# fenghansen/YOND_public

Hardware: AMD Instinct MI355X
Metric: Bayer megapixels/sec end-to-end (NLE+VST+denoise+iVST) (higher is better)
Workload: dtype f32 (3x3 convolutions: f32 operands as two f16 halves -- 22-23 significant bits -- on the f16 MFMA, 3 products per f32 product, f32 accumulate; per-layer error vs float64 asserted <= 2x the f32 direct kernel's and <= 2e-5 of max|ref| (tests/test_hip_conv.py; measured 1.3e-6 vs 1.5e-6), whole frame v

## Files before the change

yond_public_amd/csrc/common.h:

```cpp
#pragma once
#include <hip/hip_runtime.h>
#include <stdint.h>
#include "../../include/yond_hip.h"

#ifdef YOND_EXPERIMENTS
#include <stdlib.h>
static inline long yond_exp_long(const char* name, long dflt) {
    const char* e = getenv(name);
    return e ? atol(e) : dflt;
}
#else
#define yond_exp_long(name, dflt) (dflt)
#endif

typedef float f32x16 __attribute__((ext_vector_type(16)));
typedef float f32x4 __attribute__((ext_vector_type(4)));
typedef float f32x2 __attribute__((ext_vector_type(2)));

#define YOND_LAUNCH_CHECK()                          \
    do {                                             \
        hipError_t e__ = hipGetLastError();          \
        if (e__ != hipSuccess) return (int)e__;      \
    } while (0)

struct YondRange {
    int pos = 0;
    unsigned neg = 0;
    __device__ __forceinline__ void add(const f32x4& v) {
        const int b0 = __float_as_int(v[0]), b1 = __float_as_int(v[1]), b2 = __float_as_int(v[2]), b3 = __float_as_int(v[3]);
        pos = max(max(max(pos, b0), b1), max(b2, b3));
        neg = max(max(max(neg, (unsigned)b0), (unsigned)b1), max((unsigned)b2, (unsigned)b3));
    }
    __device__ __forceinline__ bool at_most(float limit) const {
        return pos <= __float_as_int(limit) && neg <= (0x80000000u | (unsigned)__float_as_int(limit));
    }
    __device__ __forceinline__ bool below(float limit) const {
        return pos < __float_as_int(limit) && neg < (0x80000000u | (unsigned)__float_as_int(limit));
    }
};

__device__ __forceinline__ float silu_f(float x) { return x / (1.0f + expf(-x)); }

__device__ __forceinline__ int reflect101(int i, int n) {
    if (n == 1) return 0;
    const int period = 2 * (n - 1);
    i %= period;
    if (i < 0) i += period;
    return i >= n ? period - i : i;
}

__device__ __forceinline__ float wave_max(float v) {
#pragma unroll
    for (int o = 32; o > 0; o >>= 1) v = fmaxf(v, __shfl_xor(v, o));
    return v;
}

__device__ __forceinline__ double wave_sum(double v) {
#pragma unroll
    for (int o = 32; o > 0; o >>= 1) v += __shfl_xor(v, o);
    return v;
}

template <int I>
struct IntC {
// ... 10 lines not shown
```

yond_public_amd/csrc/conv_split.hip:

```cpp
#include "conv_split_kernel.h"

SPLIT_GROUP_K1S2(SPLIT_EXTERN)
SPLIT_GROUP_S1_64(SPLIT_EXTERN)
SPLIT_GROUP_S1_32(SPLIT_EXTERN)
SPLIT_GROUP_HALF(SPLIT_EXTERN)
SPLIT_GROUP_HALF128(SPLIT_EXTERN)
SPLIT_GROUP_HALF_TALL(SPLIT_EXTERN)
SPLIT_GROUP_FOLD(SPLIT_EXTERN)
SPLIT_GROUP_FOLD_S2(SPLIT_EXTERN)
SPLIT_GROUP_FOLD_K1(SPLIT_EXTERN)
SPLIT_GROUP_FOLD_NHWC(SPLIT_EXTERN)
SPLIT_GROUP_K1_D2(SPLIT_EXTERN)
SPLIT_GROUP_OSP(SPLIT_EXTERN)
SPLIT_GROUP_ISP(SPLIT_EXTERN)
SPLIT_GROUP_ISP_OSP(SPLIT_EXTERN)
SPLIT_GROUP_ISP_K1S2(SPLIT_EXTERN)
SPLIT_GROUP_K1_SUB2(SPLIT_EXTERN)
SPLIT_GROUP_WRES(SPLIT_EXTERN)
SPLIT_GROUP_D2(SPLIT_EXTERN)
SPLIT_GROUP_H_OSP(SPLIT_EXTERN)
SPLIT_GROUP_H_ISP_OSP(SPLIT_EXTERN)
SPLIT_GROUP_H_ISP_O4(SPLIT_EXTERN)
SPLIT_GROUP_H_K1S2(SPLIT_EXTERN)
SPLIT_GROUP_H_D2(SPLIT_EXTERN)
// ... 220 lines not shown
            if (half128s2) {
                if (!tall) return YOND_EUNSUPPORTED;
                return d.dst2 ? YOND_EUNSUPPORTED : launch_split<2, 8, 128, 2, 1, 2, false, false, false, 2>(d, st);
            }
            if (tall) return d.dst2 ? launch_split<2, 8, 64, 2, 1, 2, false, false, false, 2, false, false, true>(d, st) : launch_split<2, 8, 64, 2, 1, 2, false, false, false, 2>(d, st);
            return d.dst2 ? launch_split<2, 4, 64, 1, 1, 2, false, false, false, 2, false, false, true>(d, st) : launch_split<2, 4, 64, 1, 1, 2, false, false, false, 2>(d, st);
        }
#ifdef YOND_EXPERIMENTS
        if (isp && parts == 2 && yond_exp_long("YOND_SPLIT_S2_ROLES", 0) != 0)
            return d.dst2 ? launch_split<2, 4, 64, 2, 2, 2, false, false, false, 2, false, false, true, 0, 8, 1>(d, st) : launch_split<2, 4, 64, 2, 2, 2, false, false, false, 2, false, false, false, 0, 8, 1>(d, st);
        if (isp && parts == 2 && yond_exp_long("YOND_SPLIT_S2_W4", 0) != 0)
            return d.dst2 ? launch_split<2, 4, 64, 2, 2, 2, false, false, false, 2, false, false, true, 0, 4>(d, st) : launch_split<2, 4, 64, 2, 2, 2, false, false, false, 2, false, false, false, 0, 4>(d, st);
#endif
        if (isp && d.dst2) return launch_split<2, 4, 64, 1, 2, 2, false, false, false, 2, false, false, true>(d, st);
        if (isp) return launch_split<2, 4, 64, 1, 2, 2, false, false, false, 2>(d, st);
        if (!isp && parts == 2 && d.Wo <= 16 && !d.src1 && !d.res && !d.in_fmt && !d.out_fmt && yond_exp_long("YOND_SPLIT_FOLD", 1) != 0) {
            const int f = d.Wo <= 8 ? 4 : 2;
            const long long subs = (long long)d.N * ((d.Ho + 3) / 4) * ((d.Wo + 32 / f - 1) / (32 / f));
            const long long tiles_f = (long long)(d.Cout / 64) * ((subs + f - 1) / f), tiles = (long long)(d.Cout / 64) * ((d.Ho + 3) / 4) * d.N;
            if ((tiles_f + 255) / 256 < (tiles + 255) / 256)
                return f == 2 ? launch_split<2, 4, 64, 1, 2, 2, false, false, false, 0, false, false, false, 2>(d, st) : launch_split<2, 4, 64, 1, 2, 2, false, false, false, 0, false, false, false, 4>(d, st);
        }
        return parts == 2 ? launch_split<2, 4, 64, 1, 2, 2, false>(d, st) : launch_split<2, 4, 64, 1, 1, 2, false>(d, st);
    }
    if (d.Ho != d.H || d.Wo != d.W) return YOND_EINVAL;
    if (d.out4_dst && (tn != 32 || (parts != 2 && !isp))) return YOND_EUNSUPPORTED;
    if (op4) return YOND_EUNSUPPORTED;
    long long tiles12 = (long long)(d.Cout / 64) * ((d.Wo + 31) / 32) * ((d.Ho + 11) / 12) * d.N;
    {
        const long long tiles8 = (long long)(d.Cout / 64) * ((d.Wo + 31) / 32) * ((d.Ho + 7) / 8) * d.N;
        const long long r12 = (tiles12 + 255) / 256, r8 = (tiles8 + 255) / 256;
        if (8000 * r8 < 10044 * r12) tiles12 = 0;
    }
    const bool wres = parts == 2 && tn == 32 && d.Cout == 32 && d.C0 + d.C1 == 32 && yond_exp_long("YOND_SPLIT_WRES", 1) != 0;
#ifdef YOND_EXPERIMENTS
    const bool w4 = wres && (long long)((d.Wo + 31) / 32) * ((d.Ho + 7) / 8) * d.N >= 2048 && yond_exp_long("YOND_SPLIT_L0_W4", 0) != 0;
    if (w4 && isp && osp && !d.out4_dst) return launch_split<1, 8, 32, 2, 2, 2, false, false, false, true, true, false, false, 0, 4>(d, st);
    if (w4 && isp && !osp && d.out4_dst) return launch_split<1, 8, 32, 2, 2, 2, false, true, false, true, false, false, false, 0, 4>(d, st);
    if (w4 && !isp && osp && d.pre_act && !d.out4_dst) return launch_split<1, 8, 32, 2, 2, 2, true, false, false, false, true, false, false, 0, 4>(d, st);
#endif
    if (wres && isp && osp && !d.out4_dst) return launch_split<1, 16, 32, 2, 2, 2, false, false, false, true, true>(d, st);
    if (wres && isp && !osp && d.out4_dst) return launch_split<1, 16, 32, 2, 2, 2, false, true, false, true, false>(d, st);
    if (wres && !isp && osp && d.pre_act && !d.out4_dst) return launch_split<1, 16, 32, 2, 2, 2, true, false, false, false, true>(d, st);
    if ((isp || osp) && parts == 1) {
        if (osp && d.out4_dst) return YOND_EUNSUPPORTED;
        if (!isp && !(osp && d.pre_act)) return YOND_EUNSUPPORTED;
        if (isp && !osp) return (d.out4_dst && tn == 32) ? launch_split<1, 16, 32, 2, 1, 3, false, true, false, true>(d, st) : YOND_EUNSUPPORTED;
        if (half128) return isp ? launch_split<1, 8, 128, 2, 1, 3, false, false, false, true, true>(d, st) : launch_split<1, 8, 128, 2, 1, 3, true, false, false, false, true>(d, st);
        const bool t4_64 = tn == 64 && (long long)(d.Cout / 64) * ((d.Wo + 31) / 32) * ((d.Ho + 15) / 16) * d.N >= 256;
        const bool t4_32 = tn == 32 && (long long)((d.Wo + 31) / 32) * ((d.Ho + 31) / 32) * d.N >= 256;
        if (isp) {
            if (t4_64) return launch_split<1, 16, 64, 4, 1, 2, false, false, false, true, true>(d, st);
            if (t4_32) return launch_split<1, 32, 32, 4, 1, 2, false, false, false, true, true>(d, st);
            if (tn == 64 && tiles12 >= 256) return launch_split<1, 12, 64, 3, 1, 2, false, false, false, true, true>(d, st);
            if (tn == 64) return launch_split<1, 8, 64, 2, 1, 3, false, false, false, true, true>(d, st);
            return launch_split<1, 16, 32, 2, 1, 3, false, false, false, true, true>(d, st);
        }
        if (t4_64) return launch_split<1, 16, 64, 4, 1, 2, true, false, false, false, true>(d, st);
        if (tn == 64 && tiles12 >= 256) return launch_split<1, 12, 64, 3, 1, 2, true, false, false, false, true>(d, st);
        if (tn == 64) return launch_split<1, 8, 64, 2, 1, 3, true, false, false, false, true>(d, st);
        return launch_split<1, 16, 32, 2, 1, 3, true, false, false, false, true>(d, st);
    }
    if (isp || osp) {
        if (osp && d.out4_dst) return YOND_EUNSUPPORTED;
        int fold = 0;
        if (osp && (isp || d.pre_act) && tn == 64 && parts == 2 && d.Wo <= 16 && d.Wo == d.W && d.Ho == d.H && !d.src1 && yond_exp_long("YOND_SPLIT_FOLD", 1) != 0) {
            const int f = d.Wo <= 8 ? 4 : 2;
            const long long subs = (long long)d.N * ((d.Ho + 3) / 4) * ((d.Wo + 32 / f - 1) / (32 / f));
            const long long tiles_f = (long long)(d.Cout / 64) * ((subs + f - 1) / f), tiles8 = (long long)(d.Cout / 64) * ((d.Ho + 7) / 8) * d.N;
            const bool fits = (long long)d.H * d.W * (d.C0 > d.Cout ? d.C0 : d.Cout) * 4 * f < (1LL << 31);
            if (fits && 2 * ((tiles_f + 255) / 256) < 3 * ((tiles8 + 255) / 256)) fold = f;
        }
        if (isp && osp) {
            if (fold == 2) return launch_split<1, 4, 64, 1, 2, 3, false, false, false, true, true, false, false, 2>(d, st);
            if (fold == 4) return launch_split<1, 4, 64, 1, 2, 3, false, false, false, true, true, false, false, 4>(d, st);
            if (tn == 64 && tiles12 >= 256) return launch_split<1, 12, 64, 3, 2, 2, false, false, false, true, true>(d, st);
            if (tn == 64) return launch_split<1, 8, 64, 2, 2, 3, false, false, false, true, true>(d, st);
            return launch_split<1, 16, 32, 2, 2, 3, false, false, false, true, true>(d, st);
        }
        if (osp) {
            if (fold == 2) return launch_split<1, 4, 64, 1, 2, 3, true, false, false, false, true, false, false, 2>(d, st);
            if (fold == 4) return launch_split<1, 4, 64, 1, 2, 3, true, false, false, false, true, false, false, 4>(d, st);
            if (tn == 64 && tiles12 >= 256) return d.pre_act ? launch_split<1, 12, 64, 3, 2, 2, true, false, false, false, true>(d, st) : launch_split<1, 12, 64, 3, 2, 2, false, false, false, false, true>(d, st);
            if (tn == 64) return d.pre_act ? launch_split<1, 8, 64, 2, 2, 3, true, false, false, false, true>(d, st) : launch_split<1, 8, 64, 2, 2, 3, false, false, false, false, true>(d, st);
            return d.pre_act ? launch_split<1, 16, 32, 2, 2, 3, true, false, false, false, true>(d, st) : launch_split<1, 16, 32, 2, 2, 3, false, false, false, false, true>(d, st);
        }
        if (tn == 64 && tiles12 >= 256) return launch_split<1, 12, 64, 3, 2, 2, false, false, false, true>(d, st);
        if (tn == 64) return launch_split<1, 8, 64, 2, 2, 3, false, false, false, true>(d, st);
        if (d.out4_dst) return launch_split<1, 16, 32, 2, 2, 3, false, true, false, true>(d, st);
        return launch_split<1, 16, 32, 2, 2, 3, false, false, false, true>(d, st);
    }
    if (half128) {
        if (d.Ho != d.H || d.Wo != d.W) return YOND_EINVAL;
        long long t12 = (long long)(d.Cout / 128) * ((d.Wo + 31) / 32) * ((d.Ho + 11) / 12) * d.N;
        const long long t8 = (long long)(d.Cout / 128) * ((d.Wo + 31) / 32) * ((d.Ho + 7) / 8) * d.N;
        if (8000 * ((t8 + 255) / 256) < 10044 * ((t12 + 255) / 256)) t12 = 0;
        if (t12 >= 256) return d.pre_act ? launch_split<1, 12, 128, 3, 1, 2, true>(d, st) : launch_split<1, 12, 128, 3, 1, 2, false>(d, st);
        return d.pre_act ? launch_split<1, 8, 128, 2, 1, 3, true>(d, st) : launch_split<1, 8, 128, 2, 1, 3, false>(d, st);
    }
    if (tn == 64) {
        const bool th12 = tiles12 >= 256;
        if (parts == 2 && !d.pre_act && !d.src1 && !d.in_fmt && !d.out_fmt && !d.res_fmt && !d.out4_dst && !(d.ebatch && (d.escale || d.eshift)) && d.Wo <= 16 &&
            yond_exp_long("YOND_SPLIT_FOLD", 1) != 0) {
            const int f = d.Wo <= 8 ? 4 : 2;
// ... 20 lines not shown
```

yond_public_amd/csrc/conv_split_kernel.h:

```cpp
#pragma once
#include "common.h"
#include <cstdlib>

typedef _Float16 f16x8 __attribute__((ext_vector_type(8)));
typedef _Float16 f16x4 __attribute__((ext_vector_type(4)));

#ifndef SPLIT_DBG
#define SPLIT_DBG 0
#endif
#if SPLIT_DBG
static __device__ unsigned long long g_split_dbg[2][64][12];
#ifdef SPLIT_DBG_READER
extern "C" int SPLIT_DBG_READER(unsigned long long* host) {
    return (int)hipMemcpyFromSymbol(host, HIP_SYMBOL(g_split_dbg), sizeof(g_split_dbg));
}
#endif
#define SDBG(slot)                                                                                  \
    do {                                                                                            \
        if (blockIdx.x == 0 && (wave == 0 || wave == 4) && lane == 0 && dbg_step < 64)              \
            g_split_dbg[wave >> 2][dbg_step][slot] = __builtin_readcyclecounter();                  \
    } while (0)
#else
#define SDBG(slot) do {} while (0)
#endif
// ... 45 lines not shown
    static constexpr int NDI = (NDS + NWAVE - 1) / NWAVE;
    static_assert(NWB == 2 || NWB == 3, "two or three weight buffers");
    static_assert(!K1 || (STRIDE == 1 && PIX_ITEMS % NT == 0), "1x1 mode: whole chunks per pass of the staging threads");
    static_assert((NWAVE == 8 || NWAVE == 4) && RG * NCW == NWC && NW >= 1 && NW * NCW * 32 == TN, "wave grid does not cover the tile");
    static_assert(!ROLES || (NWAVE == 8 && !K1 && FOLD == 0), "role split: eight waves, the 3x3 forms");
    static_assert(FOLD == 0 || FOLD == 2 || FOLD == 4, "folded tiles: two or four sub-tiles");
};

constexpr int split_gcd(int a, int b) { return b == 0 ? a : split_gcd(b, a % b); }
constexpr int split_pairs(int mw, int stride, int r) {
    int n = 0;
    for (int m = 0; m < mw; ++m) n += (r - m * stride >= 0 && r - m * stride <= 2) ? 1 : 0;
    return n;
}
__device__ __forceinline__ float split_silu(float x) {
    return x * __builtin_amdgcn_rcpf(1.0f + __builtin_amdgcn_exp2f(x * -1.44269504088896341f));
}
template <int N>
__device__ __forceinline__ void split_barrier_keep_loads() { asm volatile("s_waitcnt vmcnt(%0) lgkmcnt(0)\n\ts_barrier" ::"n"(N) : "memory"); }

template <int STRIDE, int TH, int TN, int MW, int PARTS, int NWB, bool PRE, bool O4 = false, bool K1 = false, int ISPM = 0, bool OSP = false, bool S2 = false, bool D2 = false, int FOLD = 0, int NWAVE = 8, int ROLES = 0>
__global__ __launch_bounds__(64 * NWAVE, (NWAVE == 4 && STRIDE == 1) ? 2 : 1) void conv_split_kernel(const YondConvDesc d) {
    using C = SplitCfg<STRIDE, TH, TN, MW, PARTS, NWB, K1, FOLD, NWAVE, ROLES>;
    static_assert(!ROLES || (ISPM == 2 && !OSP && !O4 && !PRE), "role split: the register-staged split-plane input (stride 2)");
    static_assert(!FOLD || (!O4 && !S2 && ((!K1 && STRIDE == 1 && ISPM != 2 && OSP) || (STRIDE == 2 && (ISPM == 2 || (ISPM == 0 && !PRE && !D2))) || (K1 && ISPM == 2) || (!K1 && STRIDE == 1 && ISPM == 0 && !OSP && !PRE))),
                  "folded tiles: the split-plane data flow's kernels (3x3 stride 1: LDS-DMA or register-staged input, split-plane store; stride 2 and the decoder GEMM: register-staged split planes) "
                  "and the plain [N][H][W][C] 3x3 layer (training, UNetSeeInDark)");
    constexpr bool ISP = ISPM == 1, ISR = ISPM == 2;
    static_assert(ISPM == 0 || !PRE, "split-plane input: the producer applied the activation");
    static_assert(!OSP || (!O4 && !K1 && STRIDE == 1), "split-plane output: 3x3 stride-1 layers");
    static_assert(!S2 || (K1 && ISPM == 2 && TN == 64), "two sub-positions per tile: the decoder GEMM with register-staged split planes");
    static_assert(!D2 || (!OSP && !O4 && ((!K1 && STRIDE == 2) || (K1 && ISPM == 2 && !S2 && TN == 64))), "second output: the stride-2 layers and the decoder GEMM at split precision");
    constexpr int NACC = PARTS;
    constexpr int IPP = ISR ? 2 * PARTS : 4;
    constexpr int PIX_ITEMS = C::IH * C::IW * IPP;
    constexpr int NITEM = C::NPT * PIX_ITEMS;
    static_assert(!K1 || PIX_ITEMS % C::NTS == 0, "1x1 mode: whole chunks per pass of the staging threads");
    constexpr int NIN = ISP ? 0 : (NITEM + C::NTS - 1) / C::NTS;
    constexpr int NINA = NIN > 0 ? NIN : 1;
    constexpr int NDI = ISP ? C::NDI : 0;
    constexpr int KD = K1 ? PIX_ITEMS / C::NTS : NIN;
    constexpr int DPER = C::WPP / split_gcd(C::WPP, NWAVE);
    constexpr int NG = ISP ? (NDI < DPER ? NDI : DPER) : KD;
    constexpr int NOPS = C::NWT + NIN + NDI;
    constexpr int KEEP = (ISP || ROLES) ? (C::WAHEAD == 2 ? C::NWT_MIN : 0) : (C::WAHEAD == 2 ? NIN + C::NWT_MIN : NIN);
    extern __shared__ __attribute__((aligned(16))) float smem[];

    const int tid = threadIdx.x, lane = tid & 63, wave = tid >> 6;
    const int stid = ROLES ? tid - C::NTS : tid;
    const bool consumer = !ROLES || __builtin_amdgcn_readfirstlane(wave) < C::NWC;
    const int li = lane & 31, lh = lane >> 5;
    constexpr int FSW = FOLD ? 32 / FOLD : 32;
    const int fsub = FOLD ? li / FSW : 0, fcol = FOLD ? li % FSW : li, flds = (FOLD && !K1) ? li + (STRIDE == 2 ? 1 : 2) * fsub : li;
    const int rg = wave % C::RG, cg = wave / C::RG;

    const int nct = d.Cout / TN;
    const bool computes = d.Cout > 0;
    const int fnsx = (d.Wo + FSW - 1) / FSW, fnsy = (d.Ho + TH - 1) / TH;
    const int fper = fnsy * fnsx, fsubs = d.N * fper;
    struct FGeo { int n, oy0, ox0; };
    auto fold_geo = [&](int u) {
        FGeo g;
        const bool ok = u < fsubs;
        const int uu = ok ? u : fsubs - 1;
        g.n = uu / fper;
        const int r = uu - g.n * fper, ry = r / fnsx;
// ... 4 lines not shown
    const int ntx = FOLD ? (fsubs + FOLD - 1) / FOLD : (d.Wo + 31) / 32, nty = FOLD ? 1 : (d.Ho + TH - 1) / TH;
    const int Neff = FOLD ? 1 : d.N;
    const int tiles_per_img = nct * ntx * nty;
    const int total = tiles_per_img * Neff;
    const int G = gridDim.x;
    const int lslot = (G % 8 == 0) ? (blockIdx.x % 8) * (G / 8) + blockIdx.x / 8 : blockIdx.x;
    const int Cin = d.C0 + d.C1;
    const int nchunk = Cin / C::KSTEP;
    const int Cr = K1 ? d.Cout / 4 : d.Cout;
    const int cpb = S2 ? Cr / 32 : 1;
    auto k1_sp = [&](int ct, int cu) -> int {
        if constexpr (S2) return 2 * (ct / cpb) + ((cu >> 5) & 1);
        return cu / Cr;
    };
    auto k1_cb = [&](int ct, int cu) -> int {
        if constexpr (S2) return (ct % cpb) * 32 + (cu & 31);
        return cu % Cr;
    };
    const int my_sl = stid & (IPP - 1);
    const int my_plane = (my_sl >> 1) * PARTS * C::PLANE + (my_sl & 1) * 2;

    int in_lds[NINA];
#pragma unroll
    for (int k = 0; k < NIN; ++k) {
        const int it = stid + k * C::NTS;
        const int pt = it / PIX_ITEMS;
        const int pix = (it % PIX_ITEMS) / IPP;
        const int py = pix / C::IW, px = pix % C::IW;
        const int lp = (STRIDE == 2) ? py * C::TWP + (px & 1) * C::HALF + (px >> 1) : py * C::TWP + px;
        in_lds[k] = my_plane + (it < NITEM ? pt * 2 * PARTS * C::PLANE + lp * 4 : C::IH * C::TWP * 4);
        if constexpr (ISR) in_lds[k] = my_sl * C::PLANE + (it < NITEM ? pt * 2 * PARTS * C::PLANE + lp * 4 : C::IH * C::TWP * 4);
    }

    struct Tile {
        int ct, n, ox0, oy0;
        int fu0;
        int goff[NG];
        int goff1[K1 ? NG : 1];
    };
    const int wave_s = __builtin_amdgcn_readfirstlane(wave);
    const int PS0 = yond_sp_plane_units(d.H, d.W);
    const int PS1 = K1 ? yond_sp_plane_units(2 * d.H, 2 * d.W) : PS0;
    struct Cur { int tile, ch, ct, tx, ty, n; };
    int g_ct, g_tx, g_ty, g_n;
    {
        int b = G;
        g_ct = b % nct; b /= nct;
        g_tx = b % ntx; b /= ntx;
        g_ty = b % nty; g_n = b / nty;
    }
    auto cursor_at = [&](int t) {
        Cur c;
        c.tile = t; c.ch = 0;
        int b = t;
        c.ct = b % nct; b /= nct;
        c.tx = b % ntx; b /= ntx;
        c.ty = b % nty; c.n = b / nty;
        return c;
    };
    const bool rev = d.tile_order != 0;
    auto tile_origin = [&](const Cur& c, Tile& T) {
        T.n = rev ? Neff - 1 - c.n : c.n;
        T.ct = c.ct;
        T.ox0 = (rev ? ntx - 1 - c.tx : c.tx) * 32;
        T.oy0 = (rev ? nty - 1 - c.ty : c.ty) * TH;
        T.fu0 = 0;
        if constexpr (FOLD != 0) {
            T.fu0 = FOLD * (rev ? ntx - 1 - c.tx : c.tx);
            const FGeo g = fold_geo(T.fu0);
            T.n = g.n; T.oy0 = g.oy0; T.ox0 = g.ox0;
        }
    };
    auto decode = [&](const Cur& c, Tile& T) {
        tile_origin(c, T);
        const int n = T.n;
        if constexpr (ISP) {
#pragma unroll
            for (int k = 0; k < NG; ++k) {
                const int sid = k * NWAVE + wave_s;
                const int q = (sid % C::WPP) * 64 + lane;
                const int py = q / C::TWP, rem = q % C::TWP;
                const int px = STRIDE == 2 ? 2 * (rem % C::HALF) + rem / C::HALF : rem;
                const bool valid = q < C::UPP && px < C::IW;
                int gy = K1 ? T.oy0 + py : T.oy0 * STRIDE - 1 + py, gx = K1 ? T.ox0 + px : T.ox0 * STRIDE - 1 + px;
                int nshift = 0;
                if constexpr (FOLD != 0) {
                    const int sb = px / C::FSUBW, lx = px - C::FSUBW * sb;
                    const FGeo g = fold_geo(T.fu0 + sb);
                    gy = g.oy0 >= d.Ho ? -1 : g.oy0 - 1 + py;
                    gx = g.ox0 - 1 + lx;
                    nshift = (g.n - T.n) * ((d.C0 / 16) * (2 * PARTS) * PS0 * 16);
                }
                const bool in = gy >= 0 && gy < d.H && gx >= 0 && gx < d.W;
                T.goff[k] = !valid ? -1 : (in ? (gy * d.W + gx) * 16 + nshift : (d.H * d.W) * 16);
                if constexpr (K1) {
                    const int sp = k1_sp(T.ct, T.ct * TN);
                    T.goff1[k] = !valid ? -1 : (in ? (2 * gy + (sp >> 1)) * (2 * d.W) + 2 * gx + (sp & 1) : 4 * d.H * d.W) * 16;
                }
            }
        } else {
        int tid_g = stid;
        if constexpr (ISPM == 0 && !OSP && !K1) asm volatile("" : "+v"(tid_g));
#pragma unroll
        for (int k = 0; k < KD; ++k) {
            const int it = tid_g + k * C::NTS;
            const int pix = (it % PIX_ITEMS) / IPP;
            const int py = pix / C::IW, px = pix % C::IW;
            int gy = K1 ? T.oy0 + py : T.oy0 * STRIDE - 1 + py, gx = K1 ? T.ox0 + px : T.ox0 * STRIDE - 1 + px;
            int nb = n * d.H * d.W;
            int ushift = 0, ushift1 = 0;
            if constexpr (FOLD != 0) {
                constexpr int SUBW = K1 ? FSW : C::FSUBW;
                const int sb = px / SUBW, lx = px - SUBW * sb;
                const FGeo g = fold_geo(T.fu0 + sb);
                gy = g.oy0 >= d.Ho ? -1 : (K1 ? g.oy0 + py : g.oy0 * STRIDE - 1 + py);
                gx = K1 ? g.ox0 + lx : g.ox0 * STRIDE - 1 + lx;
                ushift1 = (g.n - n) * (d.C1 / 16) * (2 * PARTS) * PS1;
                nb = d.in_fmt == YOND_FMT_PLANES4 ? nb + (g.n - n) * (d.C0 / 4) * d.H * d.W : g.n * d.H * d.W;
                ushift = (g.n - n) * (d.C0 / 16) * (2 * PARTS) * PS0;
            }
            const bool ok = it < NITEM && gy >= 0 && gy < d.H && gx >= 0 && gx < d.W;
            T.goff[k] = ok ? (nb + gy * d.W + gx) : -1;
            if constexpr (ISR) T.goff[k] = ok ? gy * d.W + gx + ushift : d.H * d.W;
            if constexpr (K1) {
                const int sp = k1_sp(T.ct, T.ct * TN);
                T.goff1[k] = ok ? ((n * 2 * d.H + 2 * gy + (sp >> 1)) * (2 * d.W) + 2 * gx + (sp & 1)) : -1;
                if constexpr (ISR) T.goff1[k] = ok ? (2 * gy + (sp >> 1)) * (2 * d.W) + 2 * gx + (sp & 1) + ushift1 : 4 * d.H * d.W;
            }
        }
        }
    };

    constexpr int NSET = ROLES ? 1 : (MW >= 3 || (STRIDE == 2 && PARTS == 1 && TN == 128)) ? 2 : 3;
    static_assert(NSET == 3 || C::WAHEAD == 1, "the two-set pipeline goes with two weight buffers");
    f32x4 vin[NSET][NINA];
    unsigned vin_ok[NSET] = {};
    YondRange amax;
    struct LoadSrc { const float* src[C::NPT]; int A[C::NPT], B[C::NPT]; bool hi[C::NPT]; int dx[C::NPT]; };
    const bool in_p4 = d.in_fmt == YOND_FMT_PLANES4;
    auto load_src = [&](int ch, int n) {
        LoadSrc L;
#pragma unroll
        for (int t = 0; t < C::NPT; ++t) {
            const int c0 = (ch * C::NPT + t) * C::KC;
            const bool second = c0 >= d.C0;
            int Cs = second ? d.C1 : d.C0, cc = second ? c0 - d.C0 : c0;
            L.src[t] = second ? d.src1 : d.src0;
            L.hi[t] = second && K1;
            L.dx[t] = 0;
            if constexpr (S2) {
                if (second) {
                    const int creal = Cr;
                    const int q = cc / creal;
                    L.dx[t] = q == 1 ? 1 : 0;
                    cc = q < 2 ? cc - q * creal : 0;
                    Cs = creal;
                }
            }
            if constexpr (ISR) {
                L.A[t] = 4;
                L.B[t] = ((n * (Cs / 16) + cc / 16) * (2 * PARTS) + my_sl) * (L.hi[t] ? PS1 : PS0) * 4;
            } else if (in_p4) {
                const int hw = d.H * d.W * (L.hi[t] ? 4 : 1);
                L.A[t] = 4;
                L.B[t] = 4 * ((n * (Cs / 4) + cc / 4 + my_sl) * hw - n * hw);
            } else {
                L.A[t] = Cs;
                L.B[t] = cc + my_sl * 4;
            }
        }
        return L;
    };
    auto issue_load = [&](auto pc, auto kc, const Tile& T, const LoadSrc& L) {
        constexpr int P = decltype(pc)::value, k = decltype(kc)::value;
        constexpr int t = K1 ? (k * C::NTS) / PIX_ITEMS : 0;
        constexpr int kd = k % KD;
        const bool ok = T.goff[kd] >= 0;
        int po = T.goff[kd];
        if constexpr (K1) po = L.hi[t] ? T.goff1[kd] : po;
        if constexpr (S2) {
            if (L.hi[t] && L.dx[t] && T.goff1[kd] != 4 * d.H * d.W) po += 1;
        }
        vin[P][k] = *(const f32x4*)(L.src[t] + (long long)(ok ? po : 0) * L.A[t] + L.B[t]);
        if (k == 0) vin_ok[P] = 0;
        vin_ok[P] |= (ok ? 1u : 0u) << k;
    };
    constexpr bool W_IS_SCRATCH = TN >= 64 && !K1 && STRIDE == 1 && !OSP;
    const bool wres = NWB == 2 && !W_IS_SCRATCH && nchunk == 2 && nct == 1;
    bool wskip = false;
    auto issue_dma = [&](auto kc, const float* wsrc, float* wbuf) {
        constexpr int k = decltype(kc)::value;
        if (wskip) return;
        const unsigned lds0 = (unsigned)(uintptr_t)(__attribute__((address_space(3))) float*)wbuf;
        const int it = stid + k * C::NTS;
        const int it_wave = __builtin_amdgcn_readfirstlane(it - lane);
        const unsigned lds_wave = __builtin_amdgcn_readfirstlane(lds0 + (unsigned)it_wave * 16u);
        const unsigned voff = (unsigned)it * 16u;
        if (C::NWV % C::NTS == 0 || it_wave < C::NWV)
            asm volatile("s_mov_b32 m0, %0\n\ts_nop 0\n\tglobal_load_lds_dwordx4 %1, %2" ::"s"(lds_wave), "v"(voff), "s"(wsrc) : "memory");
    };
    struct InSrc { const char* base[C::NPT]; unsigned hi; };
    auto in_src = [&](int ch, int n) {
        InSrc I;
        I.hi = 0;
#pragma unroll
        for (int t = 0; t < C::NPT; ++t) {
            const int c0 = (ch * C::NPT + t) * C::KC;
            const bool second = c0 >= d.C0;
            const bool hi = K1 && second;
            const int c16 = (second ? c0 - d.C0 : c0) / 16, nc16 = (second ? d.C1 : d.C0) / 16;
            const char* src = (const char*)(second ? d.src1 : d.src0);
            const unsigned long long a = (unsigned long long)(uintptr_t)(src + (size_t)(n * nc16 + c16) * (2 * PARTS) * (size_t)(hi ? PS1 : PS0) * 16);
            const unsigned lo = __builtin_amdgcn_readfirstlane((unsigned)a), hi32 = __builtin_amdgcn_readfirstlane((unsigned)(a >> 32));
            I.base[t] = (const char*)(uintptr_t)(((unsigned long long)hi32 << 32) | lo);
            I.hi |= (hi ? 1u : 0u) << t;
        }
        return I;
    };
    auto issue_in_dma = [&](auto kc, const Tile& T, const InSrc& I, float* ob) {
        constexpr int k = decltype(kc)::value;
        const int sid = k * NWAVE + wave_s;
        const int plane = sid / C::WPP, wv = sid - plane * C::WPP;
        const int pt = plane / (2 * PARTS), pl = plane - pt * (2 * PARTS);
        const bool hi = K1 && ((I.hi >> pt) & 1u);
        const unsigned lds0 = (unsigned)(uintptr_t)(__attribute__((address_space(3))) float*)ob;
        const unsigned lds_wave = __builtin_amdgcn_readfirstlane(lds0 + (unsigned)(plane * C::PLANE * 4 + wv * 1024));
        const char* b0 = I.base[0];
        if constexpr (C::NPT > 1) b0 = pt == 1 ? I.base[1] : (pt == 2 ? I.base[C::NPT - 1] : b0);
        const unsigned long long ga = (unsigned long long)(uintptr_t)(b0 + (size_t)pl * (size_t)(hi ? PS1 : PS0) * 16);
        const unsigned ga_lo = __builtin_amdgcn_readfirstlane((unsigned)ga), ga_hi = __builtin_amdgcn_readfirstlane((unsigned)(ga >> 32));
        const char* gb = (const char*)(uintptr_t)(((unsigned long long)ga_hi << 32) | ga_lo);
        int voff = T.goff[k % NG];
        if constexpr (K1) voff = hi ? T.goff1[k % NG] : voff;
        if (sid < C::NDS && voff >= 0)
            asm volatile("s_mov_b32 m0, %0\n\ts_nop 0\n\tglobal_load_lds_dwordx4 %1, %2" ::"s"(lds_wave), "v"(voff), "s"(gb) : "memory");
    };
    auto weight_src = [&](int ct, int ch) {
        const unsigned long long a = (unsigned long long)(uintptr_t)(d.wpk + ((size_t)ct * nchunk + ch) * C::W_FLOATS);
        const unsigned lo = __builtin_amdgcn_readfirstlane((unsigned)a), hi = __builtin_amdgcn_readfirstlane((unsigned)(a >> 32));
        return (const float*)(uintptr_t)(((unsigned long long)hi << 32) | lo);
    };
    constexpr int NE = 4 * NIN;
    auto stage_task = [&](auto pc, auto ec, float* ob) {
        constexpr int P = decltype(pc)::value;
        constexpr int e = decltype(ec)::value, k = e / 4, j = e % 4;
        if constexpr (ISR) {
            if constexpr (j == 3) *(f32x4*)(ob + in_lds[k]) = vin[P][k];
            return;
        }
        float x = vin[P][k][j];
        if (PRE) x = split_silu(x);
        vin[P][k][j] = ((vin_ok[P] >> k) & 1u) ? x : 0.0f;
        if constexpr (j == 3) {
            const f32x4 v = vin[P][k];
            amax.add(v);
            const f16x4 h = {(_Float16)v[0], (_Float16)v[1], (_Float16)v[2], (_Float16)v[3]};
            *(f16x4*)(ob + in_lds[k]) = h;
            if constexpr (PARTS == 2) {
                const f16x4 l = {(_Float16)((v[0] - (float)h[0]) * 2048.0f), (_Float16)((v[1] - (float)h[1]) * 2048.0f),
                                 (_Float16)((v[2] - (float)h[2]) * 2048.0f), (_Float16)((v[3] - (float)h[3]) * 2048.0f)};
                *(f16x4*)(ob + in_lds[k] + C::PLANE) = l;
            }
        }
    };
    auto write_in = [&](auto pc, float* ob) { static_for<0, NE>([&](auto ec) { stage_task(pc, ec, ob); }); };

    f32x16 acc[NACC][MW][C::NW];
    auto zero_acc = [&]() {
#pragma unroll
        for (int a = 0; a < NACC; ++a)
#pragma unroll
            for (int m = 0; m < MW; ++m)
#pragma unroll
                for (int nn = 0; nn < C::NW; ++nn)
#pragma unroll
                    for (int r = 0; r < 16; ++r) acc[a][m][nn][r] = 0.0f;
    };

    const int x_off = (lh * PARTS) * C::PLANE + ((rg * MW * (K1 ? 1 : STRIDE)) * C::TWP + flds) * 4;
    const int w_off = ((lh * PARTS) * TN + (cg * C::NW) * 32 + li) * 4;
// ... 55 lines not shown
                            wt[dx % WS][dy][nn][a == 2 ? PARTS - 1 : 0], xr[q % XD][a == 0 ? PARTS - 1 : 0], acc[a == 1 ? 0 : 1][m][nn], 0, 0, 0);
                }
            }
            if constexpr (wrep) loadW1(IntC<dx + 1>{}, IntC<wdy>{});
            if constexpr (q == 0) { if (wave_hi) __builtin_amdgcn_s_setprio(1); }
            if constexpr (q == NQ / 2) { if (wave_hi) __builtin_amdgcn_s_setprio(0); }
            if constexpr (q == Q0 - 1 && !ROLES) prep();
            if constexpr (q == NQ / 4) SDBG(8);
            if constexpr (q == NQ / 2) SDBG(9);
            if constexpr (q == (3 * NQ) / 4) SDBG(10);
            constexpr int qq = q >= Q0 ? q - Q0 : 0;
            constexpr int NQO = (ISP && C::WAHEAD == 1) ? (NQW + 1) / 2 : NQW;
            constexpr int qo = qq < NQO ? qq : NQO;
            constexpr int o_lo = (q >= Q0 && !ROLES) ? (qo * NOPS + NQO - 1) / NQO : 0, o_hi = (q >= Q0 && !ROLES) ? ((qo + 1 < NQO ? qo + 1 : NQO) * NOPS + NQO - 1) / NQO : 0;
            static_for<o_lo, o_hi>([&](auto oc) {
                constexpr int o = decltype(oc)::value;
                if constexpr (ISP) {
                    if constexpr (o < NDI) issue_in_dma(IntC<o>{}, lt, is_s, ob);
                    else issue_dma(IntC<o - NDI>{}, wsrc_s, wnext);
                } else if constexpr (C::LOADS_FIRST) {
                    if constexpr (o < NIN) issue_load(fc, IntC<o>{}, lt, ls_s);
                    else issue_dma(IntC<o - NIN>{}, wsrc_s, wnext);
                } else {
                    if constexpr (o < C::NWT) issue_dma(IntC<o>{}, wsrc_s, wnext);
                    else issue_load(fc, IntC<o - C::NWT>{}, lt, ls_s);
                }
            });
            constexpr int e_lo = (q >= Q0 && !ROLES) ? qq * NE / NQW : 0, e_hi = (q >= Q0 && !ROLES) ? (qq + 1) * NE / NQW : 0;
            static_for<e_lo, e_hi>([&](auto ec) { stage_task(pc, ec, ob); });
            constexpr int nfin = (e_hi + 0) / 4 - (e_lo + 0) / 4;
            constexpr int nrd = (q + 2 < NQ ? PARTS : 0) + (wpre ? (K1 ? 1 : 3) * C::NW * PARTS : 0);
            if constexpr (nrd > 0) __builtin_amdgcn_sched_group_barrier(0x100, nrd, 0);
            constexpr int ntr = (!ISR && PRE) ? (e_hi - e_lo) * 2 : 0;
            constexpr int nvalu = ISR ? 0 : (e_hi - e_lo) * (PRE ? 5 : 2) + nfin * (PARTS == 2 ? 22 : 6);
            constexpr int vpm = (nvalu + nmf - 1) / nmf;
#pragma unroll
            for (int i = 0; i < nmf; ++i) {
                __builtin_amdgcn_sched_group_barrier(0x008, 1, 0);
                if ((i * ntr) / nmf != ((i + 1) * ntr) / nmf) __builtin_amdgcn_sched_group_barrier(0x400, 1, 0);
                if constexpr (vpm > 0) __builtin_amdgcn_sched_group_barrier(0x002, vpm, 0);
            }
            if constexpr (wrep) __builtin_amdgcn_sched_group_barrier(0x100, C::NW * PARTS, 0);
            if constexpr (nfin > 0) __builtin_amdgcn_sched_group_barrier(0x200, ISR ? nfin : nfin * PARTS, 0);
        });
    };

    const float slope_eff = d.post_act == 2 ? d.slope : 1.0f;
    const bool silu_out = d.post_act == 1;
    constexpr int EPS = 36;
    constexpr int EP_FLOATS = NWAVE * 32 * EPS;
    constexpr bool EP_IN_W = TN >= 64 && !K1;
    constexpr bool EP_FIT = STRIDE == 1 && (C::EP_OWN || EP_FLOATS <= (EP_IN_W ? C::W_FLOATS : C::IN_FLOATS));
    f32x4 pes[C::NW], pet[C::NW];
    auto epi_prefetch = [&](const Tile& T) __attribute__((always_inline)) {
        const int u = lane & 7;
#pragma unroll
        for (int nn = 0; nn < C::NW; ++nn) {
            const int cu = T.ct * TN + (cg * C::NW + nn) * 32 + 4 * u;
            int eoff = (d.ebatch ? T.n * Cr : 0) + (K1 ? k1_cb(T.ct, cu) : cu);
            if constexpr (FOLD != 0) eoff = (d.ebatch ? fold_geo(T.fu0 + (lane >> 4)).n * Cr : 0) + cu;
            if constexpr (OSP) {
                const float* src = (lane & 8) ? d.eshift : d.escale;
                pes[nn] = *(const f32x4*)(src ? src + eoff : d.wpk);
            } else {
                pes[nn] = *(const f32x4*)(d.escale ? d.escale + eoff : d.wpk);
                pet[nn] = *(const f32x4*)(d.eshift ? d.eshift + eoff : d.wpk);
            }
// ... 650 lines not shown
```

yond_public_amd/engine.py:

```python
import ctypes as C
import os

import numpy as np
import torch

from . import _lib as L


def _rup(c, m=32):
    return (c + m - 1) // m * m


def _np_ptr(a):
    return C.c_void_p(a.ctypes.data)


WINO_DEFAULT = 'split'


SPLIT_PLANES = True
SP_FLOW = True
HALF_FLOW = True
HALF_K1_TN128 = True
HALF_S2_TN128 = True
# ... 253 lines not shown
            return False
        prec = getattr(self, 'precision', 'fp32')
        if prec not in ('fp32', 'fp16'):
            return False
        parts = 2 if prec == 'fp32' else 1
        return all(pc.ksize == 3 and pc.stride == 1 and pc.split(parts) is not None for pc in (pc1, pc2))

    def _sp_flow(self, N, H, W):
        if not (SPLIT_PLANES and SP_FLOW) or getattr(self, 'strict', False) or getattr(self, 'conv_algo', WINO_DEFAULT) != 'split':
            return False
        prec = getattr(self, 'precision', 'fp32')
        if prec not in ('fp32', 'fp16') or (prec == 'fp16' and not HALF_FLOW) or sp_plane_units(H, W) * 64 * 4 >= 2 ** 31:
            return False
        parts = 2 if prec == 'fp32' else 1
        for i, blk in self.blocks.items():
            for k in ('conv1', 'conv2', 'pool', 'upsc'):
                if k in blk and blk[k].split(parts, wide=False) is None:
                    return False
        return self._out4_fusable(self.blocks[9]['conv2'], flow=True)

    def _out4_fusable(self, pc, flow=False):
        prec = getattr(self, 'precision', 'fp32')
        return (not getattr(self, 'strict', False) and getattr(self, 'conv_algo', WINO_DEFAULT) == 'split' and (prec == 'fp32' or (prec == 'fp16' and flow))
                and pc.ksize == 3 and pc.stride == 1 and pc.gemm_n == 32 and pc.split(2 if prec == 'fp32' else 1) is not None and FUSE_OUT4)

    def _new_sp(self, key, N, H, W, Cc, parts=2):
        cache = self.__dict__.setdefault('_sp_cache', {})
        k = (key, N, H, W, Cc, parts, getattr(self, 'lane', 0))
        if k not in cache:
            cache[k] = torch.zeros(N * (Cc // 16) * 2 * parts * sp_plane_units(H, W) * 4, dtype=torch.float32, device=self.dev)
        return cache[k]

    def _conv(self, pc, src0, src1, N, H, W, dst, escale=None, eshift=None, ebatch=0, res=None, pre_act=0, post_act=0,
              slope=0.0, algo=None, out4=None, in_fmt=0, out_fmt=0, res_fmt=0, dst2=None):
        d = L.YondConvDesc()
        d.src0 = src0.data_ptr()
        d.src1 = src1.data_ptr() if src1 is not None else None
        d.C0 = pc.psplits[0]
        d.C1 = pc.psplits[1] if len(pc.psplits) > 1 else 0
        d.N, d.H, d.W = N, H, W
        if pc.stride == 2:
            d.Ho, d.Wo = (H + 1) // 2, (W + 1) // 2
        else:
            d.Ho, d.Wo = H, W
        d.Cout = pc.gemm_n
        d.ksize, d.stride, d.shuffle = pc.ksize, pc.stride, int(pc.shuffle)
        d.pre_act, d.post_act, d.slope = pre_act, post_act, slope
        prec = getattr(self, 'precision', 'fp32')
        if getattr(self, 'strict', False) and algo is None:
            prec, algo = 'fp32-mfma', 1
        if algo is None:
            algo = getattr(self, 'conv_algo', WINO_DEFAULT)
            if prec == 'fp32-mfma' and algo == 'split':
                algo = 1
            if prec == 'fp16' and WINO_DEFAULT == 'split':
                algo = 'half'
        fp16 = prec == 'fp16' or algo == 'fp16'
        wino = split = None
        if algo in ('split', 'half'):
            ws2 = (HALF_S2_TN128 and algo == 'half' and pc.stride == 2 and in_fmt == 1 and out_fmt == 2 and dst2 is None
                   and (pc.gemm_n // 128) * ((d.Wo + 31) // 32) * ((d.Ho + 7) // 8) * N >= 256)
            ws2 = ws2 or (HALF_K1_TN128 and algo == 'half' and pc.ksize == 1 and in_fmt == 1 and dst2 is None)
            split = pc.split(2 if algo == 'split' else 1, wide=(not (in_fmt or out_fmt or res_fmt or dst2 is not None)) or (HALF_FLOW_TN128 and out_fmt == 1),
                             wide_s2=ws2)
            if algo == 'half' and pc.ksize == 1 and in_fmt != 1:
                split = None
            if split is None and not fp16 and pc.ksize == 3:
                wino = pc.wino()
        elif not fp16:
            wino = pc.wino() if algo in (1, 2) else None
        if split is not None:
            tn, wpk = split
            kc = 16
            d.algo = 3 if algo == 'split' else 4
        elif wino is not None:
            tn, wpk = wino
            kc = 8
            d.algo = 1
        elif algo == 'split' and pc.ksize == 1 and not fp16 and pc.config(N, d.Ho, d.Wo, split=True)[2] is not None:
            tn, kc, wpk = pc.config(N, d.Ho, d.Wo, split=True)
            d.algo = 5
        else:
            tn, kc, wpk = pc.config(N, d.Ho, d.Wo)
            d.algo = 2 if (fp16 and pc.wmax <= 65504.0) else 0
        d.wpk = wpk.data_ptr()
        d.tn = tn
        d.kc = kc
        d.escale = escale.data_ptr() if escale is not None else None
        d.eshift = (eshift if eshift is not None else pc.bias).data_ptr()
        d.ebatch = ebatch
        d.res = res.data_ptr() if res is not None else None
        d.dst = dst.data_ptr() if dst is not None else None
        status = getattr(self, 'status', None)
        d.status = status.data_ptr() + 4 * self.status_slot if status is not None else None
        d.in_fmt, d.out_fmt, d.res_fmt = in_fmt, out_fmt, res_fmt
        d.dst2 = dst2.data_ptr() if dst2 is not None else None
        if SNAKE_ORDER and d.algo in (3, 4):
            self._tile_order = 1 - getattr(self, '_tile_order', 0)
            d.tile_order = self._tile_order
        clk = getattr(self, 'clk', None)
        d.clk = clk.data_ptr() if (clk is not None and d.algo in (3, 4)) else None
        if (in_fmt or out_fmt or res_fmt) and d.algo not in (3, 4):
            raise L.YondHipError("split-plane / 4-channel-plane tensors need the split-operand kernel (algo 3, or 4 with h-only planes)")
        if out4 is not None:
            w4, b4, x4, ub4, o4 = out4
            if d.algo not in (3, 4):
                raise L.YondHipError("fused output projection needs the split-operand 3x3 kernel")
            d.out4_w, d.out4_b = w4.data_ptr(), (b4.data_ptr() if b4 is not None else None)
            d.out4_x = x4.data_ptr() if x4 is not None else None
            d.out4_ub = ub4.data_ptr() if ub4 is not None else None
            d.out4_dst = o4.data_ptr()
        prof = getattr(self, 'prof', None)
        if prof is not None:
            tag = f"conv_wino_kernel<{tn}>" if d.algo == 1 else f"conv_mfma_kernel<{pc.ksize},{pc.stride},8,{tn},{kc}>"
            if d.algo in (3, 4):
                tag = f"conv_split_kernel<{pc.stride if pc.ksize == 3 else 'k1'},{tn},{5 - d.algo}>"
            if d.algo == 2:
                tag += "/f16"
            if d.algo == 5:
                tag += "/split"
            only = getattr(self, 'prof_only', None)
            if only is not None and not only(tag):
                prof = None
            every = getattr(self, 'prof_every', 1)
            if every > 1 and getattr(self, '_fwd_idx', 0) % every:
                prof = None
        if prof is not None:
            e0, e1 = torch.cuda.Event(enable_timing=True), torch.cuda.Event(enable_timing=True)
            e0.record()
        L.check(self.lib.yond_conv2d_f32(C.byref(d), L.stream()), "yond_conv2d_f32")
        if prof is not None:
            e1.record()
# ... 267 lines not shown
```

Baseline: 2587.

## Add fast buffer-load input path with cheaper split staging for pre-activation split conv

Adds a FASTIN specialization of the split-operand 3x3 kernel for the pre-activated, split-output, 16x32 tile configuration. It precomputes per-thread relative offsets, loads input with raw buffer loads whose out-of-range offsets return zero, and splits values into f16 hi/lo halves with fma_mix instructions instead of the generic staging path. It also adds a tile_rows flag through tile_order bit 2 that forces 12-row tiles and disables folding. The goal is fewer address and bounds-check instructions and fewer VALU operations in the input staging. The cost is more code-path complexity and size assumptions on the input, guarded by a byte-range check.

New measurement: 2604 (median of 6 runs). No clear change (+0.7%).

```diff
diff --git a/yond_public_amd/csrc/common.h b/yond_public_amd/csrc/common.h
--- a/yond_public_amd/csrc/common.h
+++ b/yond_public_amd/csrc/common.h
@@ -30,6 +30,11 @@
         const int b0 = __float_as_int(v[0]), b1 = __float_as_int(v[1]), b2 = __float_as_int(v[2]), b3 = __float_as_int(v[3]);
         pos = max(max(max(pos, b0), b1), max(b2, b3));
         neg = max(max(max(neg, (unsigned)b0), (unsigned)b1), max((unsigned)b2, (unsigned)b3));
+    }
+    __device__ __forceinline__ void add_chain(const f32x4& v) {
+        const int b0 = __float_as_int(v[0]), b1 = __float_as_int(v[1]), b2 = __float_as_int(v[2]), b3 = __float_as_int(v[3]);
+        pos = max(max(max(max(pos, b0), b1), b2), b3);
+        neg = max(max(max(max(neg, (unsigned)b0), (unsigned)b1), (unsigned)b2), (unsigned)b3);
     }
     __device__ __forceinline__ bool at_most(float limit) const {
         return pos <= __float_as_int(limit) && neg <= (0x80000000u | (unsigned)__float_as_int(limit));
diff --git a/yond_public_amd/csrc/conv_split.hip b/yond_public_amd/csrc/conv_split.hip
--- a/yond_public_amd/csrc/conv_split.hip
+++ b/yond_public_amd/csrc/conv_split.hip
@@ -276,6 +276,9 @@
         const long long r12 = (tiles12 + 255) / 256, r8 = (tiles8 + 255) / 256;
         if (8000 * r8 < 10044 * r12) tiles12 = 0;
     }
+    if (d.tile_order & 2) tiles12 = 256;
+    const bool fastin = parts == 2 && !isp && osp && d.pre_act && !d.out4_dst;
+    const bool fastin_ok = (long long)d.H * d.W * (ip4 ? 16 : (d.C0 > d.C1 ? d.C0 : d.C1)) * 4 < 0xfffffff0LL && (ip4 || !d.src1 || d.C0 == d.C1);
     const bool wres = parts == 2 && tn == 32 && d.Cout == 32 && d.C0 + d.C1 == 32 && yond_exp_long("YOND_SPLIT_WRES", 1) != 0;
 #ifdef YOND_EXPERIMENTS
     const bool w4 = wres && (long long)((d.Wo + 31) / 32) * ((d.Ho + 7) / 8) * d.N >= 2048 && yond_exp_long("YOND_SPLIT_L0_W4", 0) != 0;
@@ -285,7 +288,7 @@
 #endif
     if (wres && isp && osp && !d.out4_dst) return launch_split<1, 16, 32, 2, 2, 2, false, false, false, true, true>(d, st);
     if (wres && isp && !osp && d.out4_dst) return launch_split<1, 16, 32, 2, 2, 2, false, true, false, true, false>(d, st);
-    if (wres && !isp && osp && d.pre_act && !d.out4_dst) return launch_split<1, 16, 32, 2, 2, 2, true, false, false, false, true>(d, st);
+    if (wres && fastin && fastin_ok) return launch_split<1, 16, 32, 2, 2, 2, true, false, false, false, true>(d, st);
     if ((isp || osp) && parts == 1) {
         if (osp && d.out4_dst) return YOND_EUNSUPPORTED;
         if (!isp && !(osp && d.pre_act)) return YOND_EUNSUPPORTED;
@@ -314,6 +317,7 @@
             const long long tiles_f = (long long)(d.Cout / 64) * ((subs + f - 1) / f), tiles8 = (long long)(d.Cout / 64) * ((d.Ho + 7) / 8) * d.N;
             const bool fits = (long long)d.H * d.W * (d.C0 > d.Cout ? d.C0 : d.Cout) * 4 * f < (1LL << 31);
             if (fits && 2 * ((tiles_f + 255) / 256) < 3 * ((tiles8 + 255) / 256)) fold = f;
+            if (d.tile_order & 2) fold = 0;
         }
         if (isp && osp) {
             if (fold == 2) return launch_split<1, 4, 64, 1, 2, 3, false, false, false, true, true, false, false, 2>(d, st);
diff --git a/yond_public_amd/csrc/conv_split_kernel.h b/yond_public_amd/csrc/conv_split_kernel.h
--- a/yond_public_amd/csrc/conv_split_kernel.h
+++ b/yond_public_amd/csrc/conv_split_kernel.h
@@ -101,6 +101,9 @@
     static_assert(!S2 || (K1 && ISPM == 2 && TN == 64), "two sub-positions per tile: the decoder GEMM with register-staged split planes");
     static_assert(!D2 || (!OSP && !O4 && ((!K1 && STRIDE == 2) || (K1 && ISPM == 2 && !S2 && TN == 64))), "second output: the stride-2 layers and the decoder GEMM at split precision");
     constexpr int NACC = PARTS;
+    constexpr bool FASTIN = PRE && OSP && !O4 && !K1 && ISPM == 0 && !S2 && !D2 && FOLD == 0 && PARTS == 2 && NWAVE == 8 && ROLES == 0 && STRIDE == 1 && NWB == 2 &&
+                            TH == 16 && TN == 32;
+    constexpr int FI_MARK = (int)0xfffffff0u;
     constexpr int IPP = ISR ? 2 * PARTS : 4;
     constexpr int PIX_ITEMS = C::IH * C::IW * IPP;
     constexpr int NITEM = C::NPT * PIX_ITEMS;
@@ -171,6 +174,16 @@
         if constexpr (ISR) in_lds[k] = my_sl * C::PLANE + (it < NITEM ? pt * 2 * PARTS * C::PLANE + lp * 4 : C::IH * C::TWP * 4);
     }
 
+    const bool in_p4 = d.in_fmt == YOND_FMT_PLANES4;
+    const unsigned fi_pa = in_p4 ? 16u : 4u * (unsigned)d.C0;
+    unsigned fi_rel[NINA];
+    if constexpr (FASTIN) {
+#pragma unroll
+        for (int k = 0; k < NIN; ++k) {
+            const int pix = (stid + k * C::NTS) / IPP;
+            fi_rel[k] = (unsigned)((pix / C::IW) * d.W + pix % C::IW) * fi_pa + (unsigned)my_sl * (in_p4 ? 16u * (unsigned)(d.H * d.W) : 16u);
+        }
+    }
     struct Tile {
         int ct, n, ox0, oy0;
         int fu0;
@@ -197,7 +210,7 @@
         c.ty = b % nty; c.n = b / nty;
         return c;
     };
-    const bool rev = d.tile_order != 0;
+    const bool rev = (d.tile_order & 1) != 0;
     auto tile_origin = [&](const Cur& c, Tile& T) {
         T.n = rev ? Neff - 1 - c.n : c.n;
         T.ct = c.ct;
@@ -235,6 +248,22 @@
                 if constexpr (K1) {
                     const int sp = k1_sp(T.ct, T.ct * TN);
                     T.goff1[k] = !valid ? -1 : (in ? (2 * gy + (sp >> 1)) * (2 * d.W) + 2 * gx + (sp & 1) : 4 * d.H * d.W) * 16;
+                }
+            }
+        } else if constexpr (FASTIN) {
+            const int by = T.oy0 - 1, bx = T.ox0 - 1;
+            const unsigned tb = (unsigned)(by * d.W + bx) * fi_pa;
+            const bool interior = by >= 0 && by + C::IH <= d.H && bx >= 0 && bx + C::IW <= d.W;
+            if (interior) {
+#pragma unroll
+                for (int k = 0; k < NIN; ++k) T.goff[k] = ((k + 1) * C::NTS <= NITEM || stid + k * C::NTS < NITEM) ? (int)(fi_rel[k] + tb) : FI_MARK;
+            } else {
+#pragma unroll
+                for (int k = 0; k < NIN; ++k) {
+                    const int it = stid + k * C::NTS, pix = it / IPP;
+                    const int gy = by + pix / C::IW, gx = bx + pix % C::IW;
+                    const bool ok = it < NITEM && (unsigned)gy < (unsigned)d.H && (unsigned)gx < (unsigned)d.W;
+                    T.goff[k] = ok ? (int)(fi_rel[k] + tb) : FI_MARK;
                 }
             }
         } else {
@@ -275,8 +304,7 @@
     f32x4 vin[NSET][NINA];
     unsigned vin_ok[NSET] = {};
     YondRange amax;
-    struct LoadSrc { const float* src[C::NPT]; int A[C::NPT], B[C::NPT]; bool hi[C::NPT]; int dx[C::NPT]; };
-    const bool in_p4 = d.in_fmt == YOND_FMT_PLANES4;
+    struct LoadSrc { const float* src[C::NPT]; int A[C::NPT], B[C::NPT]; bool hi[C::NPT]; int dx[C::NPT]; const float* fbase; unsigned fbytes; };
     auto load_src = [&](int ch, int n) {
         LoadSrc L;
 #pragma unroll
@@ -296,6 +324,14 @@
                     Cs = creal;
                 }
             }
+            if constexpr (FASTIN) {
+                const long long hw = (long long)d.H * d.W;
+                const float* fb = L.src[t] + (in_p4 ? (long long)(n * (Cs / 4) + cc / 4) * hw * 4 : (long long)n * hw * Cs + cc);
+                const unsigned long long a = (unsigned long long)(uintptr_t)fb;
+                const unsigned lo = __builtin_amdgcn_readfirstlane((unsigned)a), hi32 = __builtin_amdgcn_readfirstlane((unsigned)(a >> 32));
+                L.fbase = (const float*)(uintptr_t)(((unsigned long long)hi32 << 32) | lo);
+                L.fbytes = __builtin_amdgcn_readfirstlane((unsigned)(in_p4 ? 16 * hw : hw * Cs - cc) * 4u);
+            }
             if constexpr (ISR) {
                 L.A[t] = 4;
                 L.B[t] = ((n * (Cs / 16) + cc / 16) * (2 * PARTS) + my_sl) * (L.hi[t] ? PS1 : PS0) * 4;
@@ -314,6 +350,11 @@
         constexpr int P = decltype(pc)::value, k = decltype(kc)::value;
         constexpr int t = K1 ? (k * C::NTS) / PIX_ITEMS : 0;
         constexpr int kd = k % KD;
+        if constexpr (FASTIN) {
+            const __amdgpu_buffer_rsrc_t rs = __builtin_amdgcn_make_buffer_rsrc((void*)L.fbase, 0, (int)L.fbytes, 0x00020000);
+            vin[P][k] = __builtin_bit_cast(f32x4, __builtin_amdgcn_raw_buffer_load_b128(rs, T.goff[kd], 0, 0));
+            return;
+        }
         const bool ok = T.goff[kd] >= 0;
         int po = T.goff[kd];
         if constexpr (K1) po = L.hi[t] ? T.goff1[kd] : po;
@@ -380,11 +421,35 @@
         return (const float*)(uintptr_t)(((unsigned long long)hi << 32) | lo);
     };
     constexpr int NE = 4 * NIN;
+    f32x4 fi_v[FASTIN ? NINA : 1];
     auto stage_task = [&](auto pc, auto ec, float* ob) {
         constexpr int P = decltype(pc)::value;
         constexpr int e = decltype(ec)::value, k = e / 4, j = e % 4;
         if constexpr (ISR) {
             if constexpr (j == 3) *(f32x4*)(ob + in_lds[k]) = vin[P][k];
+            return;
+        }
+        if constexpr (FASTIN) {
+            float y = split_silu(vin[P][k][j]);
+            asm("" : "+v"(y));
+            fi_v[k][j] = y;
+            if constexpr (j == 3) {
+                const f32x4 v = fi_v[k];
+                amax.add_chain(v);
+                typedef _Float16 f16x2 __attribute__((ext_vector_type(2)));
+                const f16x2 h01 = {(_Float16)v[0], (_Float16)v[1]}, h23 = {(_Float16)v[2], (_Float16)v[3]};
+                const f16x4 h = {h01[0], h01[1], h23[0], h23[1]};
+                *(f16x4*)(ob + in_lds[k]) = h;
+                const float s0 = v[0] * 2048.0f, s1 = v[1] * 2048.0f, s2 = v[2] * 2048.0f, s3 = v[3] * 2048.0f, m2048 = -2048.0f;
+                f16x2 l01, l23;
+                asm("v_fma_mixlo_f16 %0, %2, %4, %5 op_sel_hi:[1,0,0]\n\t"
+                    "v_fma_mixlo_f16 %1, %3, %4, %7 op_sel_hi:[1,0,0]\n\t"
+                    "v_fma_mixhi_f16 %0, %2, %4, %6 op_sel:[1,0,0] op_sel_hi:[1,0,0]\n\t"
+                    "v_fma_mixhi_f16 %1, %3, %4, %8 op_sel:[1,0,0] op_sel_hi:[1,0,0]"
+                    : "=&v"(l01), "=&v"(l23) : "v"(h01), "v"(h23), "s"(m2048), "v"(s0), "v"(s1), "v"(s2), "v"(s3));
+                const f16x4 l = {l01[0], l01[1], l23[0], l23[1]};
+                *(f16x4*)(ob + in_lds[k] + C::PLANE) = l;
+            }
             return;
         }
         float x = vin[P][k][j];
@@ -506,7 +571,7 @@
             constexpr int nrd = (q + 2 < NQ ? PARTS : 0) + (wpre ? (K1 ? 1 : 3) * C::NW * PARTS : 0);
             if constexpr (nrd > 0) __builtin_amdgcn_sched_group_barrier(0x100, nrd, 0);
             constexpr int ntr = (!ISR && PRE) ? (e_hi - e_lo) * 2 : 0;
-            constexpr int nvalu = ISR ? 0 : (e_hi - e_lo) * (PRE ? 5 : 2) + nfin * (PARTS == 2 ? 22 : 6);
+            constexpr int nvalu = ISR ? 0 : FASTIN ? (e_hi - e_lo) * 3 + nfin * 15 : (e_hi - e_lo) * (PRE ? 5 : 2) + nfin * (PARTS == 2 ? 22 : 6);
             constexpr int vpm = (nvalu + nmf - 1) / nmf;
 #pragma unroll
             for (int i = 0; i < nmf; ++i) {
diff --git a/yond_public_amd/engine.py b/yond_public_amd/engine.py
--- a/yond_public_amd/engine.py
+++ b/yond_public_amd/engine.py
@@ -309,7 +309,7 @@
         return cache[k]
 
     def _conv(self, pc, src0, src1, N, H, W, dst, escale=None, eshift=None, ebatch=0, res=None, pre_act=0, post_act=0,
-              slope=0.0, algo=None, out4=None, in_fmt=0, out_fmt=0, res_fmt=0, dst2=None):
+              slope=0.0, algo=None, out4=None, in_fmt=0, out_fmt=0, res_fmt=0, dst2=None, tile_rows=0):
         d = L.YondConvDesc()
         d.src0 = src0.data_ptr()
         d.src1 = src1.data_ptr() if src1 is not None else None
@@ -375,6 +375,8 @@
         if SNAKE_ORDER and d.algo in (3, 4):
             self._tile_order = 1 - getattr(self, '_tile_order', 0)
             d.tile_order = self._tile_order
+        if tile_rows == 12:
+            d.tile_order |= 2
         clk = getattr(self, 'clk', None)
         d.clk = clk.data_ptr() if (clk is not None and d.algo in (3, 4)) else None
         if (in_fmt or out_fmt or res_fmt) and d.algo not in (3, 4):
```
